# see--/speech_recognition

Measured on AMD Instinct MI355X. Metric: 1s 16kHz clips/sec training throughput, higher is better.
Workload: dtype f32

## Files before the change

include/kws_hip.h:

```cpp
#ifndef KWS_HIP_H_
#define KWS_HIP_H_

#include <stdint.h>

#ifdef __cplusplus
extern "C" {
#endif
#if defined(__GNUC__) || defined(__clang__)
#pragma GCC visibility push(default)
#endif

#define KWS_OK 0
#define KWS_E_INVALID (-1)
#define KWS_E_HIP (-2)
#define KWS_E_WORKSPACE (-3)

#define KWS_ABI_VERSION 5

int kws_abi_version(void);
const char* kws_last_error(void);
int kws_device_name(char* buf, int cap);

int kws_stream_create(int cls, void** stream);
int kws_stream_destroy(void* stream);
// ... 165 lines not shown
                         const float* moving_var, float eps, int C, float* bn, void* stream);
int kws_bn_relu6_apply(const float* y, const float* bn, float* out, int64_t rows, int C, int relu6,
                       void* stream);

int kws_dwconv_fwd_f32(const float* y, const float* bn, const float* w, float* z, int B, int L_in,
                       int L_out, int C, int stride, int pad_l, void* stream);
int64_t kws_dwconv_bwd_part_floats(int B, int L_in, int C);
int kws_dwconv_bwd_f32(const float* dz, const float* y, const float* bn, const float* w, float* g,
                       float* part, int B, int L_in, int L_out, int C, int stride, int pad_l,
                       void* stream);
int kws_dwconv_bwd_bn_f32(const float* dz, const float* y, const float* bn, const float* w,
                          const float* coef, float* dy, float* part, int pass, int B, int L_in,
                          int L_out, int C, int stride, int pad_l, void* stream);
int kws_dw_bwd_finalize(const float* part, int n_parts, int64_t count, int C, float* dw,
                        float* dgamma, float* dbeta, float* coef, float* scratch, void* stream);
int kws_bn_bwd_apply(float* g, const float* y, const float* bn, const float* gamma,
                     const float* coef, int64_t rows, int C, void* stream);

int kws_dwconvk_fwd_f32(const float* y, const float* bn, const float* w, float* z, int B, int L_in, int L_out, int C,
                        int k, int stride, int pad_l, void* stream);
int kws_dwconvk_bwd_part_rows(int B, int L_in, int C, int k, int stride);
int64_t kws_dwconvk_bwd_part_floats(int B, int L_in, int C, int k, int stride);
int kws_dwconvk_bwd_f32(const float* dz, const float* y, const float* bn, const float* w, float* g, float* part, int B,
                        int L_in, int L_out, int C, int k, int stride, int pad_l, void* stream);
int kws_dwconvk_bwd_finalize(const float* part, int n_parts, int64_t count, int C, int k, float* dw, float* dgamma,
                             float* dbeta, float* coef, void* stream);
int kws_dwconvk_pw1_stats_rows(int64_t M);
int kws_dwconvk_pw1_fwd_f32(const float* z, const float* p, float* y, int64_t M, int N, float* stats_part, void* stream);
int64_t kws_dwconvk_pw1_bwd_workspace_floats(int64_t M, int N);
int kws_dwconvk_pw1_bwd_f32(const float* dy, const float* z, const float* p, float* dz, float* dp, int64_t M, int N,
// ... 110 lines not shown
```

speech_recognition_amd/_lib.py:

```python
import ctypes
import os

_HERE = os.path.dirname(os.path.abspath(__file__))
LIB_PATH = os.environ.get("KWS_LIB_PATH") or os.path.join(_HERE, "libkws_hip.so")

ABI_VERSION = 5

KWS_NET_TS_ATTENTION = 1
KWS_NET_LOG_MFCC = 2
KWS_NET_STEFFE = 3
KWS_NET_RESIDUAL = 4
KWS_NET_MFCC_AND_RAW = 5
KWS_NET_CONV_1D_FAST = 6
KWS_NET_CONV_1D_SPEC = 7
KWS_NET_CONV_1D_TIME_STACKED = 8
KWS_NET_CONV_1D_HEAVY = 9
KWS_NET_CONV_1D_GRU = 10
KWS_NET_CONV_1D_MULTI_TIME_SLICED = 11
KWS_NET_CONV_1D_SIMPLE = 12
KWS_NET_XCEPTION_ATTENTION = 13


class KwsError(RuntimeError):
    pass
# ... 141 lines not shown
    "kws_gru_fwd_f32": (_I, [_P] * 12 + [_I, _I, _I, _I, _P]),
    "kws_gru_bwd_f32": (_I, [_P] * 17 + [_I, _I, _I, _I, _P]),
    "kws_attn_gate_fwd_floats": (_I64, [_I, _I, _I, _I]),
    "kws_attn_gate_bwd_floats": (_I64, [_I, _I, _I, _I]),
    "kws_attn_gate_fwd_f32": (_I, [_P] * 12 + [_I, _I, _I, _I, _I, _P]),
    "kws_attn_gate_bwd_f32": (_I, [_P] * 14 + [_I, _I, _I, _I, _I, _P]),
    "kws_transpose_f32": (_I, [_P, _P, _I, _I, _P]),
    "kws_bn_stats_finalize": (_I, [_P, _I, _I64, _I, _P, _P, _F, _F, _P, _P, _P, _P, _P]),
    "kws_bn_infer_prepare": (_I, [_P, _P, _P, _P, _F, _I, _P, _P]),
    "kws_bn_relu6_apply": (_I, [_P, _P, _P, _I64, _I, _I, _P]),
    "kws_dwconv_fwd_f32": (_I, [_P, _P, _P, _P, _I, _I, _I, _I, _I, _I, _P]),
    "kws_dwconv_bwd_part_floats": (_I64, [_I, _I, _I]),
    "kws_dwconv_bwd_f32": (_I, [_P, _P, _P, _P, _P, _P, _I, _I, _I, _I, _I, _I, _P]),
    "kws_dwconv_bwd_bn_f32": (_I, [_P, _P, _P, _P, _P, _P, _P, _I, _I, _I, _I, _I, _I, _I, _P]),
    "kws_dw_bwd_finalize": (_I, [_P, _I, _I64, _I, _P, _P, _P, _P, _P, _P]),
    "kws_bn_bwd_apply": (_I, [_P, _P, _P, _P, _P, _I64, _I, _P]),
    "kws_rmsprop_step": (_I, [_P, _P, _P, _P, _I64, _F, _F, _F, _F, _P]),
    "kws_sgd_momentum_step": (_I, [_P, _P, _P, _P, _I64, _F, _F, _F, _P]),
    "kws_adam_step": (_I, [_P, _P, _P, _P, _P, _I64, _F, _F, _F, _F, _F, _P]),
    "kws_l2_loss": (_I, [_P, _P, _I64, _P, _P]),
    "kws_net_create": (_I, [ctypes.POINTER(NetConfig), ctypes.POINTER(_P)]),
    "kws_net_destroy": (_I, [_P]),
    "kws_net_num_params": (_I64, [_P]),
    "kws_net_num_state": (_I64, [_P]),
    "kws_net_num_tensors": (_I, [_P]),
    "kws_net_tensor_info": (_I, [_P, _I, ctypes.POINTER(TensorInfo)]),
    "kws_net_workspace_bytes": (_I64, [_P, _I, _I]),
    "kws_net_debug_view": (_I, [_P, _I, _I, _I, _I, ctypes.POINTER(_I64), ctypes.POINTER(_I64)]),
    "kws_net_predict": (_I, [_P, _P, _P, _P, _I, _P, _P, _I64, _P]),
    "kws_net_train_fwd_bwd": (_I, [_P, _P, _P, _P, _P, _I, _P, _P, _P, ctypes.c_uint64, ctypes.c_uint32,
# ... 122 lines not shown
```

speech_recognition_amd/csrc/bn.hip:

```cpp
#include "internal.h"

namespace {

constexpr int FIN_CG = 16, FIN_RG = 16;
#ifndef KWS_FIN_U
#define KWS_FIN_U 16
#endif
constexpr int FIN_U = KWS_FIN_U;

__device__ float g_zero_fin[8] = {0.f, 0.f, 0.f, 0.f, 0.f, 0.f, 0.f, 0.f};

__global__ __launch_bounds__(256) void bn_stats_finalize_kernel(const float* __restrict__ part, int n_tiles,
                                                                double inv_count, int C,
                                                                const float* __restrict__ gamma,
                                                                const float* __restrict__ beta, float eps,
                                                                float one_minus_momentum, float* moving_mean,
                                                                float* moving_var, float* __restrict__ bn) {
  __shared__ double red[2][FIN_RG][FIN_CG];
  const int cg = threadIdx.x % FIN_CG, rg = threadIdx.x / FIN_CG;
  const int c = blockIdx.x * FIN_CG + cg;
  double s = 0.0, ss = 0.0;
  if (c < C) {
    for (int t = rg; t < n_tiles; t += FIN_U * FIN_RG) {
      float a[FIN_U], b[FIN_U];
// ... 138 lines not shown
    for (int q = 0; q < 5; ++q) {
      double a = 0.0;
      for (int r = 0; r < FIN_RG; ++r) a += red[q][r][cg];
      s[q] = a;
    }
    if (dbeta) dbeta[c] = (float)s[0];
    if (dgamma) dgamma[c] = (float)s[1];
    if (coef) {
      coef[c] = (float)(s[0] * inv_count);
      coef[C + c] = (float)(s[1] * inv_count);
    }
    if (dw) {
      dw[c] = (float)s[2];
      dw[C + c] = (float)s[3];
      dw[2 * C + c] = (float)s[4];
    }
  }
}

struct DwFinBatch {
  const float* part[KWS_DW_FIN_BATCH];
  float* dw[KWS_DW_FIN_BATCH];
  int n_parts[KWS_DW_FIN_BATCH], C[KWS_DW_FIN_BATCH], blk_end[KWS_DW_FIN_BATCH];
  int n;
};
__global__ __launch_bounds__(256) void dw_grad_finalize_batch_kernel(DwFinBatch b) {
  __shared__ double red[3][FIN_RG][FIN_CG];
  int m = 0;
  while (m + 1 < b.n && (int)blockIdx.x >= b.blk_end[m]) ++m;
  const int blk = blockIdx.x - (m ? b.blk_end[m - 1] : 0);
// ... 154 lines not shown

int kws_dw_bwd_finalize(const float* part, int n_parts, int64_t count, int C, float* dw, float* dgamma, float* dbeta,
                        float* coef, float* scratch, void* stream) {
  KWS_REQUIRE(part && n_parts > 0 && count > 0 && C > 0, "dw_bwd_finalize: bad arguments");
  KwsProfScope prof("bn_finalize", 0.0, 20.0 * n_parts * C, (hipStream_t)stream);
#ifdef KWS_ABL_NO_FIN
  return KWS_OK;
#endif
  KWS_TRY(pre_reduce(part, n_parts, 5 * C, scratch, (hipStream_t)stream, &part, &n_parts));
  hipLaunchKernelGGL(dw_bwd_finalize_kernel, dim3((unsigned)ceil_div(C, FIN_CG)), dim3(FIN_CG * FIN_RG), 0, (hipStream_t)stream, part,
                     n_parts, 1.0 / (double)count, C, dw, dgamma, dbeta, coef);
  KWS_LAUNCH_CHECK("dw_bwd_finalize_kernel");
  return KWS_OK;
}

int kws_bn_bwd_apply(float* g, const float* y, const float* bn, const float* gamma, const float* coef, int64_t rows,
                     int C, void* stream) {
  return kws_bn_bwd_apply_amax(g, y, bn, gamma, coef, rows, C, nullptr, (hipStream_t)stream);
}

int kws_bn_bwd_apply_amax(float* g, const float* y, const float* bn, const float* gamma, const float* coef, int64_t rows,
                          int C, unsigned* amax, void* stream_) {
  hipStream_t stream = (hipStream_t)stream_;
  KWS_REQUIRE(g && y && bn && gamma && coef && rows > 0 && C > 0 && C % 4 == 0, "bn_bwd_apply: bad arguments");
  const int64_t n4 = rows * C / 4;
  KwsProfScope prof("bn_bwd_apply", 6.0 * rows * C, 12.0 * rows * C, (hipStream_t)stream);
  hipLaunchKernelGGL(bn_bwd_apply_kernel, dim3((unsigned)ceil_div64(n4, 256)), dim3(256), 0, (hipStream_t)stream, g, y,
                     bn, gamma, coef, n4, C, amax);
  KWS_LAUNCH_CHECK("bn_bwd_apply_kernel");
  return KWS_OK;
// ... 4 lines not shown
```

speech_recognition_amd/csrc/dw_bwd_body.h:

```cpp
#pragma once
#include "internal.h"

namespace kws_dw {

#ifndef KWS_DW_NT
#define KWS_DW_NT 1
#endif
typedef float dw_v4f __attribute__((ext_vector_type(4)));
__device__ __forceinline__ float4 ld4_stream(const float* p) {
  if (KWS_DW_NT & 2) {
    const dw_v4f v = __builtin_nontemporal_load(reinterpret_cast<const dw_v4f*>(p));
    return make_float4(v.x, v.y, v.z, v.w);
  }
  return *reinterpret_cast<const float4*>(p);
}
__device__ __forceinline__ void st4_stream(float* p, float4 o) {
  if (KWS_DW_NT & 1) {
    dw_v4f v = {o.x, o.y, o.z, o.w};
    __builtin_nontemporal_store(v, reinterpret_cast<dw_v4f*>(p));
    return;
  }
  *reinterpret_cast<float4*>(p) = o;
}

// ... 10 lines not shown
}
__device__ __forceinline__ float4 f4_zero() { return make_float4(0.f, 0.f, 0.f, 0.f); }

#ifndef DW_BWD_THREADS
#define DW_BWD_THREADS 512
#endif
#ifndef DW_BWD_HT
#define DW_BWD_HT 8
#endif
#ifndef DW_BWD2_THREADS
#define DW_BWD2_THREADS 512
#endif
#ifndef DW_BWD_PARTS
#define DW_BWD_PARTS 256
#endif

struct BwdArgs {
  const float* dz; const float* y; const float* bn; const float* w; const float* coef;
  float* g; float* part;
  int B, Lin, Lout, C, pad_l, nchunks, R, Cb;
  unsigned* amax;
  int add_stride = 0, add_len = 0;
};
constexpr int bwd_smem_floats(int mode, int threads) { return mode == 2 ? 4 : 5 * threads * 4; }

template <int S, bool HAS_BN, int MODE, bool GUARD, bool ADDS = false>
__device__ __forceinline__ void bwd_body(const BwdArgs& p, float* const red, const int bid, const int nblk, const int by) {
  const float* __restrict__ dz = p.dz;
  const float* __restrict__ y = p.y;
  const float* __restrict__ bn = p.bn;
  const float* __restrict__ w = p.w;
  const float* __restrict__ coef = p.coef;
  float* __restrict__ g = p.g;
  float* __restrict__ part = p.part;
  const int B = p.B, Lin = p.Lin, Lout = p.Lout, C = p.C, pad_l = p.pad_l, nchunks = p.nchunks, R = p.R, Cb = p.Cb;
  constexpr int RSTRIDE = (MODE == 2 ? 4 : DW_BWD_THREADS * 4);
  float gmax = 0.f;
  const int C4 = Cb >> 2;
  const int tid = threadIdx.x;
  const bool live = !GUARD || tid < R * C4;
  const int r = live ? tid / C4 : 0, c4 = live ? tid - r * C4 : 0;
  const int c = by * Cb + c4 * 4;
  float4 sg = f4_zero(), sgx = f4_zero(), sw0 = f4_zero(), sw1 = f4_zero(), sw2 = f4_zero();
  float4 sc = f4_zero(), sh = f4_zero(), mean = f4_zero(), rstd = f4_zero();
  if (HAS_BN) {
    sc = *reinterpret_cast<const float4*>(bn + c);
    sh = *reinterpret_cast<const float4*>(bn + C + c);
    mean = *reinterpret_cast<const float4*>(bn + 2 * C + c);
    rstd = *reinterpret_cast<const float4*>(bn + 3 * C + c);
  }
  const float4 w0 = *reinterpret_cast<const float4*>(w + c);
  const float4 w1 = *reinterpret_cast<const float4*>(w + C + c);
  const float4 w2 = *reinterpret_cast<const float4*>(w + 2 * C + c);
  float4 c1 = f4_zero(), c2 = f4_zero();
  if (MODE == 2) {
    c1 = *reinterpret_cast<const float4*>(coef + c);
    c2 = *reinterpret_cast<const float4*>(coef + C + c);
  }
  for (int64_t ub = bid; ub * R < (int64_t)B * nchunks; ub += nblk) {
    const int64_t unit = ub * R + r;
    const int64_t b = unit / nchunks;
    const int chunk = (int)(unit - b * nchunks);
    if (b >= B || !live) continue;
    const float* yb = y + b * (int64_t)Lin * C + c;
    float* gb = g + b * (int64_t)Lin * C + c;
    const float* dzb = dz + b * (int64_t)Lout * C + c;
    const int u0 = chunk * TT;
    constexpr int HT = DW_BWD_HT;
    constexpr int ND = S == 1 ? HT + 2 : HT / 2 + 2;
    const bool podd = (pad_l & 1) != 0;
#pragma unroll
    for (int h = 0; h < TT / HT; ++h) {
      const int ub = u0 + h * HT;
      if (ub >= Lin) break;
      float4 yv[HT], D[ND];
#pragma unroll
      for (int i = 0; i < HT; ++i) yv[i] = ld4_stream(yb + (int64_t)(ub + i < Lin ? ub + i : ub) * C);
      const int t_lo = S == 1 ? ub + pad_l - 2 : ((ub + pad_l) >> 1) - 1;
#pragma unroll
      for (int j = 0; j < ND; ++j) {
        const int t = t_lo + j;
        D[j] = ld4_stream(dzb + (int64_t)(t < 0 ? 0 : (t < Lout ? t : Lout - 1)) * C);
      }
// ... 11 lines not shown
          d0 = D[i + 2]; d1 = D[i + 1]; d2 = D[i];
        } else if ((i & 1) == 0) {
          d0 = podd ? f4_zero() : D[i / 2 + 1];
          d2 = podd ? f4_zero() : D[i / 2];
          d1 = podd ? D[i / 2 + 1] : f4_zero();
        } else {
          d0 = podd ? D[(i + 1) / 2 + 1] : f4_zero();
          d2 = podd ? D[(i + 1) / 2] : f4_zero();
          d1 = podd ? f4_zero() : D[(i - 1) / 2 + 1];
        }
        const float4 yy = yv[i];
        float4 a = yy, mk = make_float4(1.f, 1.f, 1.f, 1.f), xh = f4_zero();
        if (HAS_BN) {
          const float4 pre = make_float4(fmaf(yy.x, sc.x, sh.x), fmaf(yy.y, sc.y, sh.y), fmaf(yy.z, sc.z, sh.z),
                                         fmaf(yy.w, sc.w, sh.w));
          a = make_float4(relu6f(pre.x), relu6f(pre.y), relu6f(pre.z), relu6f(pre.w));
          mk = make_float4((pre.x > 0.f && pre.x <= 6.f) ? 1.f : 0.f, (pre.y > 0.f && pre.y <= 6.f) ? 1.f : 0.f,
                           (pre.z > 0.f && pre.z <= 6.f) ? 1.f : 0.f, (pre.w > 0.f && pre.w <= 6.f) ? 1.f : 0.f);
          xh = make_float4((yy.x - mean.x) * rstd.x, (yy.y - mean.y) * rstd.y, (yy.z - mean.z) * rstd.z,
                           (yy.w - mean.w) * rstd.w);
        }
        float4 da = f4_mul(w0, d0);
        da = f4_fma(w1, d1, da);
        da = f4_fma(w2, d2, da);
        const float4 gv = f4_mul(da, mk);
        if (MODE == 2) {
          float4 o;
          o.x = sc.x * (gv.x - c1.x - (yy.x - mean.x) * rstd.x * c2.x);
          o.y = sc.y * (gv.y - c1.y - (yy.y - mean.y) * rstd.y * c2.y);
          o.z = sc.z * (gv.z - c1.z - (yy.z - mean.z) * rstd.z * c2.z);
          o.w = sc.w * (gv.w - c1.w - (yy.w - mean.w) * rstd.w * c2.w);
          st4_stream(gb + (int64_t)u * C, o);
          gmax = kws_abs4max(gmax, o);
          continue;
        }
        if (MODE == 0) {
          float4 o = gv;
          if (coef != nullptr) {
            if (!ADDS) {
              const float4 ad = *reinterpret_cast<const float4*>(coef + (b * (int64_t)Lin + u) * C + c);
              o = make_float4(o.x + ad.x, o.y + ad.y, o.z + ad.z, o.w + ad.w);
            } else {
              const int q = u / p.add_stride;
              const bool on = q * p.add_stride == u && q < p.add_len;
              const float4 ad = *reinterpret_cast<const float4*>(coef + (b * (int64_t)p.add_len + (on ? q : 0)) * C + c);
              o = make_float4(on ? o.x + ad.x : o.x, on ? o.y + ad.y : o.y, on ? o.z + ad.z : o.z, on ? o.w + ad.w : o.w);
            }
          }
          st4_stream(gb + (int64_t)u * C, o);
        }
        sg.x += gv.x; sg.y += gv.y; sg.z += gv.z; sg.w += gv.w;
        sgx = f4_fma(gv, xh, sgx);
        sw0 = f4_fma(d0, a, sw0);
        sw1 = f4_fma(d1, a, sw1);
        sw2 = f4_fma(d2, a, sw2);
      }
    }
  }
  if (MODE == 2) {
    if (p.amax && live) kws_absmax_commit(p.amax, gmax);
    return;
  }
  if constexpr (MODE != 2) {
  if (live) {
    *reinterpret_cast<float4*>(&red[0 * RSTRIDE + tid * 4]) = sg;
    *reinterpret_cast<float4*>(&red[1 * RSTRIDE + tid * 4]) = sgx;
    *reinterpret_cast<float4*>(&red[2 * RSTRIDE + tid * 4]) = sw0;
    *reinterpret_cast<float4*>(&red[3 * RSTRIDE + tid * 4]) = sw1;
    *reinterpret_cast<float4*>(&red[4 * RSTRIDE + tid * 4]) = sw2;
  }
  __syncthreads();
  for (int o = tid; o < 5 * Cb; o += blockDim.x) {
    const int q = o / Cb, ch = o - q * Cb;
    float s = 0.f;
    for (int rr = 0; rr < R; ++rr) s += red[q * RSTRIDE + (rr * C4) * 4 + ch];
    part[((int64_t)bid * 5 + q) * C + by * Cb + ch] = s;
  }
  }
}

constexpr int KWS_DW_BWD_MAX_PARTS = DW_BWD_PARTS;
struct BwdGeom {
  int nchunks, R, block, ny, Cb;
  int64_t grid;
};
inline bool bwd_geom_ok(int C) { return C > 0 && C % 4 == 0 && (C / 4) % ceil_div(C / 4, 256) == 0; }
inline BwdGeom bwd_geom(int B, int Lin, int C, bool parts = true) {
  BwdGeom g;
  const int threads = parts ? DW_BWD_THREADS : DW_BWD2_THREADS;
  const int max_parts = parts ? KWS_DW_BWD_MAX_PARTS : 1024;
  g.ny = ceil_div(C / 4, 256);
  g.Cb = C / g.ny;
  const int C4 = g.Cb / 4;
  g.nchunks = ceil_div(Lin, TT);
  g.R = threads / C4;
  if (g.R < 1) g.R = 1;
  g.block = g.R * C4;
  g.grid = ceil_div64((int64_t)B * g.nchunks, g.R);
  if (g.grid > max_parts) g.grid = max_parts;
  return g;
}

}
```

speech_recognition_amd/csrc/dwconv.hip:

```cpp
#include "dw_bwd_body.h"

namespace {
using namespace kws_dw;

#ifndef DW_FWD_GRID
#define DW_FWD_GRID 4096
#endif

template <int S, bool HAS_BN>
__global__ __launch_bounds__(256) void dwconv_fwd_kernel(const float* __restrict__ y, const float* __restrict__ bn,
                                                         const float* __restrict__ w, float* __restrict__ z,
                                                         int B, int Lin, int Lout, int C, int pad_l, int nchunks,
                                                         unsigned* amax) {
  const int C4 = C >> 2;
  float zmax = 0.f;
  const int64_t total = (int64_t)B * nchunks * C4;
  for (int64_t id = (int64_t)blockIdx.x * 256 + threadIdx.x; id < total; id += (int64_t)gridDim.x * 256) {
    const int c4 = (int)(id % C4);
    const int64_t rest = id / C4;
    const int chunk = (int)(rest % nchunks);
    const int64_t b = rest / nchunks;
    const int c = c4 * 4;
    float4 sc = f4_zero(), sh = f4_zero();
    if (HAS_BN) {
// ... 34 lines not shown
      o = f4_fma(w1, av[S * i + 1], o);
      o = f4_fma(w2, av[S * i + 2], o);
      st4_stream(zb + (int64_t)t * C, o);
      zmax = kws_abs4max(zmax, o);
    }
  }
  if (amax) kws_absmax_commit(amax, zmax);
}

#ifndef KWS_DW_BWD2_MINW
#define KWS_DW_BWD2_MINW 1
#endif
#ifndef KWS_DW_BWD1_MINW
#define KWS_DW_BWD1_MINW 1
#endif
template <int S, bool HAS_BN, int MODE, bool ADDS = false>
__global__ __launch_bounds__(MODE == 2 ? DW_BWD2_THREADS : DW_BWD_THREADS, MODE == 2 ? KWS_DW_BWD2_MINW : KWS_DW_BWD1_MINW) void dwconv_bwd_kernel(BwdArgs p) {
  __shared__ float red[bwd_smem_floats(MODE, DW_BWD_THREADS)];
  bwd_body<S, HAS_BN, MODE, false, ADDS>(p, red, (int)blockIdx.x, (int)gridDim.x, (int)blockIdx.y);
}

}


namespace {
template <int MODE>
int launch_dw_bwd(const float* dz, const float* y, const float* bn, const float* w, const float* coef, float* g,
                  float* part, int B, int L_in, int L_out, int C, int stride, int pad_l, hipStream_t st,
                  unsigned* amax = nullptr, int add_stride = 0, int add_len = 0) {
  const BwdGeom ge = bwd_geom(B, L_in, C, MODE != 2);
  KWS_REQUIRE(ge.grid < 0x7FFFFFFF, "dwconv_bwd: grid too large");
  dim3 gr((unsigned)ge.grid, (unsigned)ge.ny), b((unsigned)ge.block);
  BwdArgs a;
  a.dz = dz; a.y = y; a.bn = bn; a.w = w; a.coef = coef; a.g = g; a.part = part;
  a.B = B; a.Lin = L_in; a.Lout = L_out; a.C = C; a.pad_l = pad_l; a.nchunks = ge.nchunks; a.R = ge.R; a.Cb = ge.Cb; a.amax = amax;
  a.add_stride = add_stride; a.add_len = add_len;
  if (MODE == 0 && add_stride > 1) {
    if (stride == 1) hipLaunchKernelGGL((dwconv_bwd_kernel<1, false, MODE, true>), gr, b, 0, st, a);
    else hipLaunchKernelGGL((dwconv_bwd_kernel<2, false, MODE, true>), gr, b, 0, st, a);
    KWS_LAUNCH_CHECK("dwconv_bwd_kernel");
    return KWS_OK;
  }
  if (stride == 1) {
    if (bn) hipLaunchKernelGGL((dwconv_bwd_kernel<1, true, MODE>), gr, b, 0, st, a);
    else hipLaunchKernelGGL((dwconv_bwd_kernel<1, false, MODE>), gr, b, 0, st, a);
  } else {
    if (bn) hipLaunchKernelGGL((dwconv_bwd_kernel<2, true, MODE>), gr, b, 0, st, a);
    else hipLaunchKernelGGL((dwconv_bwd_kernel<2, false, MODE>), gr, b, 0, st, a);
  }
  KWS_LAUNCH_CHECK("dwconv_bwd_kernel");
  return KWS_OK;
}
}

extern "C" {

int kws_dwconv_fwd_f32(const float* y, const float* bn, const float* w, float* z, int B, int L_in, int L_out,
// ... 75 lines not shown
                               unsigned* amax, void* stream_) {
  hipStream_t stream = (hipStream_t)stream_;
  KWS_REQUIRE(dz && y && bn && w, "dwconv_bwd_bn: NULL pointer");
  KWS_REQUIRE(pass == 1 ? part != nullptr : (pass == 2 && coef != nullptr && dy != nullptr),
              "dwconv_bwd_bn: pass %d needs %s", pass, pass == 1 ? "part" : "coef and dy");
  KWS_REQUIRE(B > 0 && L_in > 0 && L_out > 0 && bwd_geom_ok(C),
              "dwconv_bwd_bn: bad shape B=%d L=%d->%d C=%d", B, L_in, L_out, C);
  KWS_REQUIRE(stride == 1 || stride == 2, "dwconv_bwd_bn: stride %d unsupported", stride);
  hipStream_t st = (hipStream_t)stream;
  KwsProfScope prof("dwconv_bwd", 12.0 * B * L_in * C,
                    4.0 * ((pass == 2 ? 2.0 : 1.0) * B * L_in * C + (double)B * L_out * C), st);
  if (pass == 1) return launch_dw_bwd<1>(dz, y, bn, w, nullptr, nullptr, part, B, L_in, L_out, C, stride, pad_l, st);
  return launch_dw_bwd<2>(dz, y, bn, w, coef, dy, nullptr, B, L_in, L_out, C, stride, pad_l, st, amax);
}

}
```

speech_recognition_amd/csrc/internal.h:

```cpp
#pragma once
#include "common.h"

struct kws_ts_tail_args {
  const float* y; const float* bn; const float* W1; const float* b1; const float* W2; const float* labels;
  float* probs; float* g; float* part; float* xd; float* fd; float* dl1; float* dl2; float* per_loss;
  float* per_correct; float* att; int B, T, C, NC; uint64_t seed; uint32_t step; float keep_prob; float label_smoothing;
  int loss_batch; int64_t row_offset; int train;
};
int kws_ts_tail_launch(const kws_ts_tail_args* p, hipStream_t st);
constexpr int KWS_SMALL_WGRAD_SLICES = 32;
int kws_small_wgrad_launch(const float* X, const float* D, float* out, float* out_bias, int B, int K, int N,
                           float* scratch, hipStream_t st);
int kws_metrics_launch(const float* per_loss, const float* per_correct, int B, float* metrics, hipStream_t st);
struct kws_tail_post_args {
  const float* X2; const float* D2; float* ws2; int K2, N2;
  const float* X1; const float* D1; float* ws1; int K1, N1;
  float* bias1;
  const float* per_loss; const float* per_correct; float* metrics;
  int B;
};
int kws_tail_post_launch(const kws_tail_post_args* a, int* S_out, hipStream_t st);
bool kws_conv1_supported(const kws_gather_t* g, const kws_gather_t* unfolded, int N);
int kws_conv1_stats_rows(int64_t M);
int kws_conv1_fwd(const float* x, const kws_gather_t* g, const kws_gather_t* unfolded, const float* W, float* y, int B, int N,
                  float* stats, hipStream_t st);
int64_t kws_conv1_wgrad_workspace_floats(int64_t M);
int kws_conv1_wgrad(const float* x, const kws_gather_t* g, const kws_gather_t* unfolded, const float* G, float* dW, int B,
                    int N, float* workspace, hipStream_t st);
int kws_conv1_wgrad_slabs(const float* x, const kws_gather_t* g, const kws_gather_t* unfolded, const float* G, float* dW, int B,
                          int N, float* workspace, const float* const* sl_ws, float* const* sl_out, const int64_t* sl_n,
                          const int* sl_S, int n_sl, hipStream_t st);
extern "C" int kws_reduce_slab_groups_f32(float* ws, int64_t n, int S, int per_group, hipStream_t st);
extern "C" int kws_reduce_slabs_f32(const float* ws, float* out, int64_t n, int S, hipStream_t st);
extern "C" int kws_dwconv_bwd_acc_f32(const float* dz, const float* y, const float* w, const float* add, float* g, float* part,
                                      int B, int L_in, int L_out, int C, int stride, int pad_l, hipStream_t st);
extern "C" int kws_dwconv_bwd_acc_strided_f32(const float* dz, const float* y, const float* w, const float* add, int add_stride, int add_len,
                                              float* g, float* part, int B, int L_in, int L_out, int C, int stride, int pad_l, hipStream_t st);
constexpr int KWS_SLAB_BATCH = 16;
extern "C" int kws_gemm_tn_slabs_f32(const float* A, const float* G, int64_t M, int K, int N, float* workspace, int* S,
                                     hipStream_t stream);
extern "C" int kws_gemm_dgrad_wgrad_f32(const float* dY, const float* WT, float* dZ, const float* Z, int64_t M, int cin, int cout,
                                        float* workspace, int* S, hipStream_t stream);
extern "C" bool kws_gather_strided_rows(const kws_gather_t* g, int* lda);
extern "C" int kws_gemm_nn_strided_f32(const float* A, int lda, const float* W, float* C, int64_t M, int K, int N, float* stats_part,
                                       hipStream_t stream);
extern "C" int kws_gemm_tn_slabs_strided_f32(const float* A, int lda, const float* G, int64_t M, int K, int N, float* workspace, int* S,
                                             hipStream_t stream);
extern "C" int kws_gemm_tn_gather_slabs_f32(const float* X, const kws_gather_t* g, const float* G, int B, int N, float* workspace, int* S,
                                            hipStream_t stream);
extern "C" int kws_reduce_slabs_batch(const float* const* ws, float* const* out, const int64_t* n, const int* S, int count,
                                      hipStream_t stream);
extern "C" int64_t kws_gemm_tn_workspace_floats(int64_t M, int K, int N);
struct SlabBatch {
// ... 58 lines not shown
      const float4 v2 = w[(int64_t)(k + 8) * n4 + i], v3 = w[(int64_t)(k + 12) * n4 + i];
      kws_add4(s0, v0); kws_add4(s1, v1); kws_add4(s2, v2); kws_add4(s3, v3);
    }
    for (; k < S; k += 4) kws_add4(s0, w[(int64_t)k * n4 + i]);
    kws_add4(s0, s1); kws_add4(s2, s3); kws_add4(s0, s2);
  }
  red[grp][col] = s0;
  __syncthreads();
  if (grp == 0 && i < n4) {
    float4 r = red[0][col];
    kws_add4(r, red[1][col]); kws_add4(r, red[2][col]); kws_add4(r, red[3][col]);
    reinterpret_cast<float4*>(b.out[m])[i] = r;
  }
}
#endif
struct KwsSlabQueue {
  const float* ws[KWS_SLAB_BATCH];
  float* out[KWS_SLAB_BATCH];
  int64_t n[KWS_SLAB_BATCH];
  int S[KWS_SLAB_BATCH];
  int count = 0;
  float* base = nullptr;
  int64_t used = 0, cap = 0;
  bool allow_pair = true;
  int flush(hipStream_t st) {
    if (count == 0) return 0;
    const int rc = kws_reduce_slabs_batch(ws, out, n, S, count, st);
    count = 0;
    used = 0;
    return rc;
  }
  int gemm(const float* A, const float* G, float* dW, int64_t M, int K, int N, hipStream_t st) {
    const int64_t need = (kws_gemm_tn_workspace_floats(M, K, N) + 63) / 64 * 64;
    if (count == KWS_SLAB_BATCH || used + need > cap) {
      const int rc = flush(st);
      if (rc) return rc;
    }
    if (need > cap) return KWS_E_WORKSPACE;
    ws[count] = base + used; out[count] = dW; n[count] = (int64_t)K * N;
    const int rc = kws_gemm_tn_slabs_f32(A, G, M, K, N, base + used, &S[count], st);
    if (rc) return rc;
    used += need;
    ++count;
    return 0;
  }
  int gemm_gather(const float* X, const kws_gather_t* g, const float* G, float* dW, int B, int N, hipStream_t st) {
    const int64_t M = (int64_t)B * g->L_out;
    const int K = g->taps * g->cin;
    const int64_t need = (kws_gemm_tn_workspace_floats(M, K, N) + 63) / 64 * 64;
    if (count == KWS_SLAB_BATCH || used + need > cap) {
      const int rc = flush(st);
      if (rc) return rc;
    }
    if (need > cap) return KWS_E_WORKSPACE;
    ws[count] = base + used; out[count] = dW; n[count] = (int64_t)K * N;
    int S_ = 0, lda = 0;
    if (kws_gather_strided_rows(g, &lda)) {
      const int rs = kws_gemm_tn_slabs_strided_f32(X, lda, G, M, K, N, base + used, &S_, st);
      if (rs < 0) return rs;
      if (rs == 0) {
        S[count] = S_;
        used += need;
        ++count;
        return 0;
      }
    }
    const int rc = kws_gemm_tn_gather_slabs_f32(X, g, G, B, N, base + used, &S_, st);
    if (rc) return rc;
    S[count] = -S_;
    used += need;
    ++count;
    return 0;
  }
  int pair(const float* dY, const float* WT, float* dZ, const float* Z, float* dW, int64_t M, int cin, int cout, hipStream_t st) {
    const int64_t need = (kws_gemm_tn_workspace_floats(M, cin, cout) + 63) / 64 * 64;
    if (count == KWS_SLAB_BATCH || used + need > cap) {
      const int rc = flush(st);
      if (rc) return rc;
    }
    if (need > cap) return KWS_E_WORKSPACE;
    const int rc = allow_pair ? kws_gemm_dgrad_wgrad_f32(dY, WT, dZ, Z, M, cin, cout, base + used, &S[count], st) : 1;
    if (rc < 0) return rc;
    if (rc == 0) {
      ws[count] = base + used; out[count] = dW; n[count] = (int64_t)cin * cout;
      used += need;
      ++count;
      return 0;
    }
    const int rc2 = kws_gemm_nn_f32(dY, WT, dZ, M, cout, cin, nullptr, st);
    if (rc2) return rc2;
    return gemm(Z, dY, dW, M, cin, cout, st);
// ... 39 lines not shown
```

speech_recognition_amd/csrc/net.hip:

```cpp
#include "net_internal.h"
#include <atomic>
#include <math.h>
#include <stdlib.h>

int64_t kws_net_add_tensor(kws_net* n, const std::string& name, std::vector<int64_t> shape, bool is_state, float l2,
                           int fan_in, int fan_out, float init) {
  kws_tensor_info_t t;
  memset(&t, 0, sizeof(t));
  snprintf(t.name, sizeof(t.name), "%s", name.c_str());
  int64_t size = 1;
  t.ndim = (int)shape.size();
  for (int i = 0; i < t.ndim; ++i) {
    t.shape[i] = shape[i];
    size *= shape[i];
  }
  t.size = size;
  t.is_state = is_state ? 1 : 0;
  t.l2 = l2;
  t.fan_in = fan_in;
  t.fan_out = fan_out;
  t.init = init;
  int64_t& cursor = is_state ? n->n_state : n->n_params;
  t.offset = cursor;
  cursor += (size + 3) / 4 * 4;
// ... 189 lines not shown
  const int n = K1f * C1;
  hipLaunchKernelGGL(fold_taps_kernel, dim3(ceil_div(n, 256)), dim3(256), 0, st, params + conv1, w1f, g.taps, g.cin,
                     g.stride_j, K1f, C1);
  KWS_LAUNCH_CHECK("fold_taps_kernel");
  return KWS_OK;
}
int TsProgram::unfold_conv1(const float* g1f, float* grads, hipStream_t st) const {
  const kws_gather_t& g = gather1;
  const int n = g.taps * g.cin * C1;
  hipLaunchKernelGGL(unfold_taps_kernel, dim3(ceil_div(n, 256)), dim3(256), 0, st, g1f, grads + conv1, g.taps, g.cin,
                     g.stride_j, C1);
  KWS_LAUNCH_CHECK("unfold_taps_kernel");
  return KWS_OK;
}

void TsProgram::make_layout(int B, bool training, Layout* lo) const {
  Bump bp;
  const int nb = (int)blocks.size();
  lo->y.assign(nb + 1, 0);
  lo->z.assign(nb, 0);
  int64_t max_y = (int64_t)B * L1 * C1, max_z = 0, max_part = 0, max_dwpart = 0, max_tn = 0;
  int maxC = C1;
  max_part = std::max((int64_t)kws_gemm_num_row_tiles((int64_t)B * L1), (int64_t)kws_conv1_stats_rows((int64_t)B * L1)) *
             2 * C1;
  max_tn = std::max(kws_gemm_tn_workspace_floats((int64_t)B * L1, K1f, C1),
                    kws_conv1_wgrad_workspace_floats((int64_t)B * L1));
  for (int i = 0; i < nb; ++i) {
    const Block& b = blocks[i];
    const int64_t M = (int64_t)B * b.Lout;
    if (M * b.cout > max_y) max_y = M * b.cout;
// ... 276 lines not shown
  KWS_TRY(kws_small_wgrad_launch(t.xd, t.dl1, grads + d1k, grads + d1b, B, T * C, T,
                                 ws + lo.swg, st));
  }
  {
    const BnRef& r = blocks[nb - 1].bn;
    KWS_TRY(kws_dw_bwd_finalize(part, B, (int64_t)B * T, r.C, nullptr, grads + r.gamma,
                                grads + r.beta, coef, red, st));
  }
  }
  if (run_head) KWS_TRY(transpose_all());
  float* Gb[2] = {ws + lo.G, ws + lo.G2};
  const float* sl_ws[KWS_SLAB_BATCH];
  float* sl_out[KWS_SLAB_BATCH];
  int64_t sl_n[KWS_SLAB_BATCH];
  int sl_S[KWS_SLAB_BATCH], n_sl = 0;
  KWS_REQUIRE(nb + 2 <= KWS_SLAB_BATCH, "net: %d blocks exceed the slab batch", nb);
  if (tail_S > 0) {
    sl_ws[n_sl] = ws + lo.swg; sl_out[n_sl] = grads + d2k; sl_n[n_sl] = (int64_t)2 * C * NC; sl_S[n_sl] = -tail_S; ++n_sl;
    sl_ws[n_sl] = ws + lo.swg1; sl_out[n_sl] = grads + d1k; sl_n[n_sl] = (int64_t)T * C * T; sl_S[n_sl] = -tail_S; ++n_sl;
  }
  const int i_hi = phase == 2 ? split - 1 : nb - 1, i_lo = phase == 1 ? split : 0;
  for (int i = i_hi; i >= i_lo; --i) {
    const Block& b = blocks[i];
    const int64_t M = (int64_t)B * b.Lout;
    float* Gcur = Gb[(i + 1) % 2];
    float* Gnext = Gb[i % 2];
    if (i == nb - 1)
      KWS_TRY(kws_bn_bwd_apply_amax(Gcur, ws + lo.y[i + 1], bn_at(i + 1), params + b.bn.gamma, coef, M, b.cout,
                                    h2 ? g_slots(i) : nullptr, st));
    bool paired = false;
    if (pair_bwd) {
// ... 7 lines not shown
    }
    if (!paired) {
    if (h2 && kws_gemm_nn_f16x2_supported(M, b.cout, b.cin))
      KWS_TRY(kws_gemm_nn_f16x2_f32(Gcur, ws + lo.WPd[i], DZ, M, b.cout, b.cin, g_slots(i), w_slots(i), nullptr, st));
    else
      KWS_TRY(kws_gemm_nn_f32(Gcur, ws + lo.WT[i], DZ, M, b.cout, b.cin, nullptr, st));
    if (h2 && kws_gemm_tn_f16x2_supported(M, b.cin, b.cout))
      KWS_TRY(kws_gemm_tn_f16x2_f32(ws + lo.z[i], Gcur, grads + b.pw, M, b.cin, b.cout, z_slots(i), g_slots(i), ws + lo.tn, st));
    else {
      sl_ws[n_sl] = ws + lo.tns[i]; sl_out[n_sl] = grads + b.pw; sl_n[n_sl] = (int64_t)b.cin * b.cout;
      KWS_TRY(kws_gemm_tn_slabs_f32(ws + lo.z[i], Gcur, M, b.cin, b.cout, ws + lo.tns[i], &sl_S[n_sl], st));
      ++n_sl;
    }
    }
    const BnRef& prev = (i == 0) ? bn1 : blocks[i - 1].bn;
    KWS_TRY(kws_dwconv_bwd_bn_f32(DZ, ws + lo.y[i], bn_at(i), params + b.dw, nullptr, nullptr, part, 1, B, b.Lin, b.Lout,
                                  b.cin, b.stride, b.pad_l, st));
    const int n_parts = (int)(kws_dwconv_bwd_part_floats(B, b.Lin, b.cin) / (5 * b.cin));
    KWS_TRY(kws_dw_bwd_finalize(part, n_parts, (int64_t)B * b.Lin, b.cin, grads + b.dw,
                                grads + prev.gamma, grads + prev.beta, coef, red, st));
    KWS_TRY(kws_dwconv_bwd_bn_amax_f32(DZ, ws + lo.y[i], bn_at(i), params + b.dw, coef, Gnext, nullptr, 2, B, b.Lin, b.Lout,
                                       b.cin, b.stride, b.pad_l, (h2 && i > 0) ? g_slots(i - 1) : nullptr, st));
  }
  const bool sum_with_conv1 = n_sl > 0 && phase != 1 && kws_conv1_supported(&gather1f, &gather1, C1) &&
                              kws_net_get_gemm_mode(net) != 1;
  if (n_sl > 0 && !sum_with_conv1) KWS_TRY(kws_reduce_slabs_batch(sl_ws, sl_out, sl_n, sl_S, n_sl, st));
  if (phase != 1) {
    const int64_t M = (int64_t)B * L1;
    (void)M;
    if (kws_conv1_supported(&gather1f, &gather1, C1)) {
      KWS_TRY(kws_conv1_wgrad_slabs(x, &gather1f, &gather1, Gb[0], grads + conv1, B, C1, ws + lo.tn,
                                    sl_ws, sl_out, sl_n, sl_S, sum_with_conv1 ? n_sl : 0, st));
    } else {
      KWS_TRY(kws_gemm_tn_gather_f32(x, &gather1f, Gb[0], ws + lo.g1f, B, C1, ws + lo.tn, st));
      KWS_TRY(unfold_conv1(ws + lo.g1f, grads, st));
    }
  }
// ... 123 lines not shown
```

Measured before the change: 233,900.

## Split depthwise-conv backward into lean BN-stat pass and fused dgrad+weight-grad pass

For small enough layers, the depthwise conv backward drops from a five-sum stats pass plus a separate dgrad pass to two kernels. A lean pass 3 computes only the two BN reduction sums, without relu6 activation recompute. Pass 4 writes dgrad and also accumulates the three weight-tap sums into per-block rows stored in the freed z buffer. Those rows are reduced later in the existing batched slab reduction, and the slab batch capacity is doubled to hold the extra entries. The aim is to cut redundant reductions and shared-memory traffic in the stats pass and the finalize cost, at the price of more register pressure in the dgrad kernel and a wider slab-reduction batch.

```diff
diff --git a/include/kws_hip.h b/include/kws_hip.h
--- a/include/kws_hip.h
+++ b/include/kws_hip.h
@@ -203,6 +203,13 @@
                           int L_out, int C, int stride, int pad_l, void* stream);
 int kws_dw_bwd_finalize(const float* part, int n_parts, int64_t count, int C, float* dw,
                         float* dgamma, float* dbeta, float* coef, float* scratch, void* stream);
+int kws_dwconv_bwd_rows(int B, int L_in, int C, int pass);
+int kws_dwconv_bwd_bn2_f32(const float* dz, const float* y, const float* bn, const float* w,
+                           const float* coef, float* dy, float* part, int pass, int B, int L_in,
+                           int L_out, int C, int stride, int pad_l, unsigned* amax, void* stream);
+int kws_dw_bwd_finalize2(const float* part, int n_parts, int64_t count, int C, float* dgamma,
+                         float* dbeta, float* coef, float* scratch, void* stream);
+int kws_dw_tap_rows_sum(const float* rows, int n_rows, int C, float* dw, void* stream);
 int kws_bn_bwd_apply(float* g, const float* y, const float* bn, const float* gamma,
                      const float* coef, int64_t rows, int C, void* stream);
 
diff --git a/speech_recognition_amd/_lib.py b/speech_recognition_amd/_lib.py
--- a/speech_recognition_amd/_lib.py
+++ b/speech_recognition_amd/_lib.py
@@ -179,6 +179,10 @@
     "kws_dwconv_bwd_f32": (_I, [_P, _P, _P, _P, _P, _P, _I, _I, _I, _I, _I, _I, _P]),
     "kws_dwconv_bwd_bn_f32": (_I, [_P, _P, _P, _P, _P, _P, _P, _I, _I, _I, _I, _I, _I, _I, _P]),
     "kws_dw_bwd_finalize": (_I, [_P, _I, _I64, _I, _P, _P, _P, _P, _P, _P]),
+    "kws_dwconv_bwd_rows": (_I, [_I, _I, _I, _I]),
+    "kws_dwconv_bwd_bn2_f32": (_I, [_P, _P, _P, _P, _P, _P, _P, _I, _I, _I, _I, _I, _I, _I, _P, _P]),
+    "kws_dw_bwd_finalize2": (_I, [_P, _I, _I64, _I, _P, _P, _P, _P, _P]),
+    "kws_dw_tap_rows_sum": (_I, [_P, _I, _I, _P, _P]),
     "kws_bn_bwd_apply": (_I, [_P, _P, _P, _P, _P, _I64, _I, _P]),
     "kws_rmsprop_step": (_I, [_P, _P, _P, _P, _I64, _F, _F, _F, _F, _P]),
     "kws_sgd_momentum_step": (_I, [_P, _P, _P, _P, _I64, _F, _F, _F, _P]),
diff --git a/speech_recognition_amd/csrc/bn.hip b/speech_recognition_amd/csrc/bn.hip
--- a/speech_recognition_amd/csrc/bn.hip
+++ b/speech_recognition_amd/csrc/bn.hip
@@ -176,6 +176,48 @@
       dw[c] = (float)s[2];
       dw[C + c] = (float)s[3];
       dw[2 * C + c] = (float)s[4];
+    }
+  }
+}
+
+__global__ __launch_bounds__(256) void dw_bwd_finalize2_kernel(const float* __restrict__ part, int n_parts, double inv_count, int C,
+                                                               float* dgamma, float* dbeta, float* coef) {
+  __shared__ double red[2][FIN_RG][FIN_CG];
+  const int cg = threadIdx.x % FIN_CG, rg = threadIdx.x / FIN_CG;
+  const int c = blockIdx.x * FIN_CG + cg;
+  double s[2] = {0, 0};
+  if (c < C) {
+    for (int t = rg; t < n_parts; t += FIN_U * FIN_RG) {
+      float a[FIN_U][2];
+#pragma unroll
+      for (int u = 0; u < FIN_U; ++u) {
+        const int tt = t + u * FIN_RG;
+        const bool ok = tt < n_parts;
+        const float* src = ok ? part + (int64_t)tt * 2 * C + c : g_zero_fin;
+#pragma unroll
+        for (int q = 0; q < 2; ++q) a[u][q] = src[ok ? q * C : q];
+      }
+#pragma unroll
+      for (int u = 0; u < FIN_U; ++u)
+#pragma unroll
+        for (int q = 0; q < 2; ++q) s[q] += (double)a[u][q];
+    }
+  }
+#pragma unroll
+  for (int q = 0; q < 2; ++q) red[q][rg][cg] = s[q];
+  __syncthreads();
+  if (rg == 0 && c < C) {
+#pragma unroll
+    for (int q = 0; q < 2; ++q) {
+      double a = 0.0;
+      for (int r = 0; r < FIN_RG; ++r) a += red[q][r][cg];
+      s[q] = a;
+    }
+    if (dbeta) dbeta[c] = (float)s[0];
+    if (dgamma) dgamma[c] = (float)s[1];
+    if (coef) {
+      coef[c] = (float)(s[0] * inv_count);
+      coef[C + c] = (float)(s[1] * inv_count);
     }
   }
 }
@@ -360,6 +402,20 @@
   return KWS_OK;
 }
 
+int kws_dw_bwd_finalize2(const float* part, int n_parts, int64_t count, int C, float* dgamma, float* dbeta, float* coef,
+                         float* scratch, void* stream) {
+  KWS_REQUIRE(part && n_parts > 0 && count > 0 && C > 0, "dw_bwd_finalize2: bad arguments");
+  KwsProfScope prof("bn_finalize", 0.0, 8.0 * n_parts * C, (hipStream_t)stream);
+#ifdef KWS_ABL_NO_FIN
+  return KWS_OK;
+#endif
+  KWS_TRY(pre_reduce(part, n_parts, 2 * C, scratch, (hipStream_t)stream, &part, &n_parts));
+  hipLaunchKernelGGL(dw_bwd_finalize2_kernel, dim3((unsigned)ceil_div(C, FIN_CG)), dim3(FIN_CG * FIN_RG), 0, (hipStream_t)stream, part,
+                     n_parts, 1.0 / (double)count, C, dgamma, dbeta, coef);
+  KWS_LAUNCH_CHECK("dw_bwd_finalize2_kernel");
+  return KWS_OK;
+}
+
 int kws_bn_bwd_apply(float* g, const float* y, const float* bn, const float* gamma, const float* coef, int64_t rows,
                      int C, void* stream) {
   return kws_bn_bwd_apply_amax(g, y, bn, gamma, coef, rows, C, nullptr, (hipStream_t)stream);
diff --git a/speech_recognition_amd/csrc/dw_bwd_body.h b/speech_recognition_amd/csrc/dw_bwd_body.h
--- a/speech_recognition_amd/csrc/dw_bwd_body.h
+++ b/speech_recognition_amd/csrc/dw_bwd_body.h
@@ -48,6 +48,13 @@
 #ifndef DW_BWD_PARTS
 #define DW_BWD_PARTS 256
 #endif
+#ifndef DW_BWD3_HT
+#define DW_BWD3_HT DW_BWD_HT
+#endif
+#ifndef DW_BWD4_THREADS
+#define DW_BWD4_THREADS 512
+#endif
+constexpr int bwd_threads(int mode) { return mode == 2 ? DW_BWD2_THREADS : mode == 4 ? DW_BWD4_THREADS : DW_BWD_THREADS; }
 
 struct BwdArgs {
   const float* dz; const float* y; const float* bn; const float* w; const float* coef;
@@ -56,7 +63,8 @@
   unsigned* amax;
   int add_stride = 0, add_len = 0;
 };
-constexpr int bwd_smem_floats(int mode, int threads) { return mode == 2 ? 4 : 5 * threads * 4; }
+constexpr int bwd_row_sums(int mode) { return mode == 2 ? 0 : mode == 3 ? 2 : mode == 4 ? 3 : 5; }
+constexpr int bwd_smem_floats(int mode, int threads) { return mode == 2 ? 4 : bwd_row_sums(mode) * threads * 4; }
 
 template <int S, bool HAS_BN, int MODE, bool GUARD, bool ADDS = false>
 __device__ __forceinline__ void bwd_body(const BwdArgs& p, float* const red, const int bid, const int nblk, const int by) {
@@ -68,7 +76,7 @@
   float* __restrict__ g = p.g;
   float* __restrict__ part = p.part;
   const int B = p.B, Lin = p.Lin, Lout = p.Lout, C = p.C, pad_l = p.pad_l, nchunks = p.nchunks, R = p.R, Cb = p.Cb;
-  constexpr int RSTRIDE = (MODE == 2 ? 4 : DW_BWD_THREADS * 4);
+  constexpr int RSTRIDE = (MODE == 2 ? 4 : bwd_threads(MODE) * 4);
   float gmax = 0.f;
   const int C4 = Cb >> 2;
   const int tid = threadIdx.x;
@@ -87,7 +95,7 @@
   const float4 w1 = *reinterpret_cast<const float4*>(w + C + c);
   const float4 w2 = *reinterpret_cast<const float4*>(w + 2 * C + c);
   float4 c1 = f4_zero(), c2 = f4_zero();
-  if (MODE == 2) {
+  if (MODE == 2 || MODE == 4) {
     c1 = *reinterpret_cast<const float4*>(coef + c);
     c2 = *reinterpret_cast<const float4*>(coef + C + c);
   }
@@ -100,7 +108,7 @@
     float* gb = g + b * (int64_t)Lin * C + c;
     const float* dzb = dz + b * (int64_t)Lout * C + c;
     const int u0 = chunk * TT;
-    constexpr int HT = DW_BWD_HT;
+    constexpr int HT = MODE == 3 ? DW_BWD3_HT : DW_BWD_HT;
     constexpr int ND = S == 1 ? HT + 2 : HT / 2 + 2;
     const bool podd = (pad_l & 1) != 0;
 #pragma unroll
@@ -142,7 +150,7 @@
         if (HAS_BN) {
           const float4 pre = make_float4(fmaf(yy.x, sc.x, sh.x), fmaf(yy.y, sc.y, sh.y), fmaf(yy.z, sc.z, sh.z),
                                          fmaf(yy.w, sc.w, sh.w));
-          a = make_float4(relu6f(pre.x), relu6f(pre.y), relu6f(pre.z), relu6f(pre.w));
+          if (MODE != 3) a = make_float4(relu6f(pre.x), relu6f(pre.y), relu6f(pre.z), relu6f(pre.w));
           mk = make_float4((pre.x > 0.f && pre.x <= 6.f) ? 1.f : 0.f, (pre.y > 0.f && pre.y <= 6.f) ? 1.f : 0.f,
                            (pre.z > 0.f && pre.z <= 6.f) ? 1.f : 0.f, (pre.w > 0.f && pre.w <= 6.f) ? 1.f : 0.f);
           xh = make_float4((yy.x - mean.x) * rstd.x, (yy.y - mean.y) * rstd.y, (yy.z - mean.z) * rstd.z,
@@ -152,7 +160,7 @@
         da = f4_fma(w1, d1, da);
         da = f4_fma(w2, d2, da);
         const float4 gv = f4_mul(da, mk);
-        if (MODE == 2) {
+        if (MODE == 2 || MODE == 4) {
           float4 o;
           o.x = sc.x * (gv.x - c1.x - (yy.x - mean.x) * rstd.x * c2.x);
           o.y = sc.y * (gv.y - c1.y - (yy.y - mean.y) * rstd.y * c2.y);
@@ -160,7 +168,7 @@
           o.w = sc.w * (gv.w - c1.w - (yy.w - mean.w) * rstd.w * c2.w);
           st4_stream(gb + (int64_t)u * C, o);
           gmax = kws_abs4max(gmax, o);
-          continue;
+          if (MODE == 2) continue;
         }
         if (MODE == 0) {
           float4 o = gv;
@@ -177,32 +185,42 @@
           }
           st4_stream(gb + (int64_t)u * C, o);
         }
-        sg.x += gv.x; sg.y += gv.y; sg.z += gv.z; sg.w += gv.w;
-        sgx = f4_fma(gv, xh, sgx);
-        sw0 = f4_fma(d0, a, sw0);
-        sw1 = f4_fma(d1, a, sw1);
-        sw2 = f4_fma(d2, a, sw2);
+        if (MODE != 4) {
+          sg.x += gv.x; sg.y += gv.y; sg.z += gv.z; sg.w += gv.w;
+          sgx = f4_fma(gv, xh, sgx);
+        }
+        if (MODE != 3) {
+          sw0 = f4_fma(d0, a, sw0);
+          sw1 = f4_fma(d1, a, sw1);
+          sw2 = f4_fma(d2, a, sw2);
+        }
       }
     }
   }
-  if (MODE == 2) {
+  if (MODE == 2 || MODE == 4) {
     if (p.amax && live) kws_absmax_commit(p.amax, gmax);
-    return;
+    if (MODE == 2) return;
   }
   if constexpr (MODE != 2) {
+  constexpr int NQ = bwd_row_sums(MODE);
   if (live) {
-    *reinterpret_cast<float4*>(&red[0 * RSTRIDE + tid * 4]) = sg;
-    *reinterpret_cast<float4*>(&red[1 * RSTRIDE + tid * 4]) = sgx;
-    *reinterpret_cast<float4*>(&red[2 * RSTRIDE + tid * 4]) = sw0;
-    *reinterpret_cast<float4*>(&red[3 * RSTRIDE + tid * 4]) = sw1;
-    *reinterpret_cast<float4*>(&red[4 * RSTRIDE + tid * 4]) = sw2;
+    int q = 0;
+    if (MODE != 4) {
+      *reinterpret_cast<float4*>(&red[(q++) * RSTRIDE + tid * 4]) = sg;
+      *reinterpret_cast<float4*>(&red[(q++) * RSTRIDE + tid * 4]) = sgx;
+    }
+    if (MODE != 3) {
+      *reinterpret_cast<float4*>(&red[(q++) * RSTRIDE + tid * 4]) = sw0;
+      *reinterpret_cast<float4*>(&red[(q++) * RSTRIDE + tid * 4]) = sw1;
+      *reinterpret_cast<float4*>(&red[(q++) * RSTRIDE + tid * 4]) = sw2;
+    }
   }
   __syncthreads();
-  for (int o = tid; o < 5 * Cb; o += blockDim.x) {
+  for (int o = tid; o < NQ * Cb; o += blockDim.x) {
     const int q = o / Cb, ch = o - q * Cb;
     float s = 0.f;
     for (int rr = 0; rr < R; ++rr) s += red[q * RSTRIDE + (rr * C4) * 4 + ch];
-    part[((int64_t)bid * 5 + q) * C + by * Cb + ch] = s;
+    part[((int64_t)bid * NQ + q) * C + by * Cb + ch] = s;
   }
   }
 }
@@ -213,10 +231,10 @@
   int64_t grid;
 };
 inline bool bwd_geom_ok(int C) { return C > 0 && C % 4 == 0 && (C / 4) % ceil_div(C / 4, 256) == 0; }
-inline BwdGeom bwd_geom(int B, int Lin, int C, bool parts = true) {
+inline BwdGeom bwd_geom(int B, int Lin, int C, int mode = 1) {
   BwdGeom g;
-  const int threads = parts ? DW_BWD_THREADS : DW_BWD2_THREADS;
-  const int max_parts = parts ? KWS_DW_BWD_MAX_PARTS : 1024;
+  const int threads = bwd_threads(mode);
+  const int max_parts = mode != 2 ? KWS_DW_BWD_MAX_PARTS : 1024;
   g.ny = ceil_div(C / 4, 256);
   g.Cb = C / g.ny;
   const int C4 = g.Cb / 4;
diff --git a/speech_recognition_amd/csrc/dwconv.hip b/speech_recognition_amd/csrc/dwconv.hip
--- a/speech_recognition_amd/csrc/dwconv.hip
+++ b/speech_recognition_amd/csrc/dwconv.hip
@@ -72,9 +72,18 @@
 #ifndef KWS_DW_BWD1_MINW
 #define KWS_DW_BWD1_MINW 1
 #endif
+#ifndef KWS_DW_BWD3_MINW
+#define KWS_DW_BWD3_MINW 1
+#endif
+#ifndef KWS_DW_BWD4_MINW
+#define KWS_DW_BWD4_MINW 1
+#endif
+constexpr int bwd_minw(int mode) {
+  return mode == 2 ? KWS_DW_BWD2_MINW : mode == 3 ? KWS_DW_BWD3_MINW : mode == 4 ? KWS_DW_BWD4_MINW : KWS_DW_BWD1_MINW;
+}
 template <int S, bool HAS_BN, int MODE, bool ADDS = false>
-__global__ __launch_bounds__(MODE == 2 ? DW_BWD2_THREADS : DW_BWD_THREADS, MODE == 2 ? KWS_DW_BWD2_MINW : KWS_DW_BWD1_MINW) void dwconv_bwd_kernel(BwdArgs p) {
-  __shared__ float red[bwd_smem_floats(MODE, DW_BWD_THREADS)];
+__global__ __launch_bounds__(bwd_threads(MODE), bwd_minw(MODE)) void dwconv_bwd_kernel(BwdArgs p) {
+  __shared__ float red[bwd_smem_floats(MODE, bwd_threads(MODE))];
   bwd_body<S, HAS_BN, MODE, false, ADDS>(p, red, (int)blockIdx.x, (int)gridDim.x, (int)blockIdx.y);
 }
 
@@ -86,19 +95,25 @@
 int launch_dw_bwd(const float* dz, const float* y, const float* bn, const float* w, const float* coef, float* g,
                   float* part, int B, int L_in, int L_out, int C, int stride, int pad_l, hipStream_t st,
                   unsigned* amax = nullptr, int add_stride = 0, int add_len = 0) {
-  const BwdGeom ge = bwd_geom(B, L_in, C, MODE != 2);
+  const BwdGeom ge = bwd_geom(B, L_in, C, MODE);
   KWS_REQUIRE(ge.grid < 0x7FFFFFFF, "dwconv_bwd: grid too large");
   dim3 gr((unsigned)ge.grid, (unsigned)ge.ny), b((unsigned)ge.block);
   BwdArgs a;
   a.dz = dz; a.y = y; a.bn = bn; a.w = w; a.coef = coef; a.g = g; a.part = part;
   a.B = B; a.Lin = L_in; a.Lout = L_out; a.C = C; a.pad_l = pad_l; a.nchunks = ge.nchunks; a.R = ge.R; a.Cb = ge.Cb; a.amax = amax;
   a.add_stride = add_stride; a.add_len = add_len;
-  if (MODE == 0 && add_stride > 1) {
+  if constexpr (MODE == 0) if (add_stride > 1) {
     if (stride == 1) hipLaunchKernelGGL((dwconv_bwd_kernel<1, false, MODE, true>), gr, b, 0, st, a);
     else hipLaunchKernelGGL((dwconv_bwd_kernel<2, false, MODE, true>), gr, b, 0, st, a);
     KWS_LAUNCH_CHECK("dwconv_bwd_kernel");
     return KWS_OK;
   }
+  if constexpr (MODE == 3 || MODE == 4) {
+    if (stride == 1) hipLaunchKernelGGL((dwconv_bwd_kernel<1, true, MODE>), gr, b, 0, st, a);
+    else hipLaunchKernelGGL((dwconv_bwd_kernel<2, true, MODE>), gr, b, 0, st, a);
+    KWS_LAUNCH_CHECK("dwconv_bwd_kernel");
+    return KWS_OK;
+  } else
   if (stride == 1) {
     if (bn) hipLaunchKernelGGL((dwconv_bwd_kernel<1, true, MODE>), gr, b, 0, st, a);
     else hipLaunchKernelGGL((dwconv_bwd_kernel<1, false, MODE>), gr, b, 0, st, a);
@@ -204,4 +219,29 @@
   return launch_dw_bwd<2>(dz, y, bn, w, coef, dy, nullptr, B, L_in, L_out, C, stride, pad_l, st, amax);
 }
 
-}
+int kws_dwconv_bwd_rows(int B, int L_in, int C, int pass) {
+  if (B <= 0 || L_in <= 0 || !bwd_geom_ok(C) || (pass != 3 && pass != 4)) return 0;
+  return (int)bwd_geom(B, L_in, C, pass).grid;
+}
+
+int kws_dwconv_bwd_bn2_f32(const float* dz, const float* y, const float* bn, const float* w, const float* coef, float* dy,
+                           float* part, int pass, int B, int L_in, int L_out, int C, int stride, int pad_l, unsigned* amax,
+                           void* stream) {
+  KWS_REQUIRE(dz && y && bn && w && part, "dwconv_bwd_bn2: NULL pointer");
+  KWS_REQUIRE(pass == 3 || (pass == 4 && coef != nullptr && dy != nullptr), "dwconv_bwd_bn2: pass %d (3, or 4 with coef and dy)", pass);
+  KWS_REQUIRE(B > 0 && L_in > 0 && L_out > 0 && bwd_geom_ok(C), "dwconv_bwd_bn2: bad shape B=%d L=%d->%d C=%d", B, L_in, L_out, C);
+  KWS_REQUIRE(stride == 1 || stride == 2, "dwconv_bwd_bn2: stride %d unsupported", stride);
+  hipStream_t st = (hipStream_t)stream;
+  KwsProfScope prof("dwconv_bwd", (pass == 3 ? 9.0 : 15.0) * B * L_in * C,
+                    4.0 * ((pass == 4 ? 2.0 : 1.0) * B * L_in * C + (double)B * L_out * C), st);
+  if (pass == 3) return launch_dw_bwd<3>(dz, y, bn, w, nullptr, nullptr, part, B, L_in, L_out, C, stride, pad_l, st);
+  return launch_dw_bwd<4>(dz, y, bn, w, coef, dy, part, B, L_in, L_out, C, stride, pad_l, st, amax);
+}
+
+int kws_dw_tap_rows_sum(const float* rows, int n_rows, int C, float* dw, void* stream) {
+  KWS_REQUIRE(rows && dw && n_rows > 0 && C > 0 && C % 4 == 0, "dw_tap_rows_sum: bad arguments");
+  const int64_t n = 3 * (int64_t)C;
+  return kws_reduce_slabs_batch(&rows, &dw, &n, &n_rows, 1, (hipStream_t)stream);
+}
+
+}
diff --git a/speech_recognition_amd/csrc/internal.h b/speech_recognition_amd/csrc/internal.h
--- a/speech_recognition_amd/csrc/internal.h
+++ b/speech_recognition_amd/csrc/internal.h
@@ -36,7 +36,7 @@
                                       int B, int L_in, int L_out, int C, int stride, int pad_l, hipStream_t st);
 extern "C" int kws_dwconv_bwd_acc_strided_f32(const float* dz, const float* y, const float* w, const float* add, int add_stride, int add_len,
                                               float* g, float* part, int B, int L_in, int L_out, int C, int stride, int pad_l, hipStream_t st);
-constexpr int KWS_SLAB_BATCH = 16;
+constexpr int KWS_SLAB_BATCH = 32;
 extern "C" int kws_gemm_tn_slabs_f32(const float* A, const float* G, int64_t M, int K, int N, float* workspace, int* S,
                                      hipStream_t stream);
 extern "C" int kws_gemm_dgrad_wgrad_f32(const float* dY, const float* WT, float* dZ, const float* Z, int64_t M, int cin, int cout,
@@ -125,6 +125,7 @@
   }
 }
 #endif
+constexpr int KWS_SLAB_QUEUE = 16;
 struct KwsSlabQueue {
   const float* ws[KWS_SLAB_BATCH];
   float* out[KWS_SLAB_BATCH];
@@ -143,7 +144,7 @@
   }
   int gemm(const float* A, const float* G, float* dW, int64_t M, int K, int N, hipStream_t st) {
     const int64_t need = (kws_gemm_tn_workspace_floats(M, K, N) + 63) / 64 * 64;
-    if (count == KWS_SLAB_BATCH || used + need > cap) {
+    if (count == KWS_SLAB_QUEUE || used + need > cap) {
       const int rc = flush(st);
       if (rc) return rc;
     }
@@ -159,7 +160,7 @@
     const int64_t M = (int64_t)B * g->L_out;
     const int K = g->taps * g->cin;
     const int64_t need = (kws_gemm_tn_workspace_floats(M, K, N) + 63) / 64 * 64;
-    if (count == KWS_SLAB_BATCH || used + need > cap) {
+    if (count == KWS_SLAB_QUEUE || used + need > cap) {
       const int rc = flush(st);
       if (rc) return rc;
     }
@@ -185,7 +186,7 @@
   }
   int pair(const float* dY, const float* WT, float* dZ, const float* Z, float* dW, int64_t M, int cin, int cout, hipStream_t st) {
     const int64_t need = (kws_gemm_tn_workspace_floats(M, cin, cout) + 63) / 64 * 64;
-    if (count == KWS_SLAB_BATCH || used + need > cap) {
+    if (count == KWS_SLAB_QUEUE || used + need > cap) {
       const int rc = flush(st);
       if (rc) return rc;
     }
diff --git a/speech_recognition_amd/csrc/net.hip b/speech_recognition_amd/csrc/net.hip
--- a/speech_recognition_amd/csrc/net.hip
+++ b/speech_recognition_amd/csrc/net.hip
@@ -227,6 +227,11 @@
   return KWS_OK;
 }
 
+#ifndef KWS_DW_LEAN_MAX_ELEMS
+#define KWS_DW_LEAN_MAX_ELEMS 14000000ll
+#endif
+static bool dw_bwd_lean(int B, int Lin, int Lout, int C) { return (int64_t)B * (Lin + Lout) * C <= KWS_DW_LEAN_MAX_ELEMS; }
+
 void TsProgram::make_layout(int B, bool training, Layout* lo) const {
   Bump bp;
   const int nb = (int)blocks.size();
@@ -533,7 +538,7 @@
   float* sl_out[KWS_SLAB_BATCH];
   int64_t sl_n[KWS_SLAB_BATCH];
   int sl_S[KWS_SLAB_BATCH], n_sl = 0;
-  KWS_REQUIRE(nb + 2 <= KWS_SLAB_BATCH, "net: %d blocks exceed the slab batch", nb);
+  KWS_REQUIRE(2 * nb + 2 <= KWS_SLAB_BATCH, "net: %d blocks exceed the slab batch", nb);
   if (tail_S > 0) {
     sl_ws[n_sl] = ws + lo.swg; sl_out[n_sl] = grads + d2k; sl_n[n_sl] = (int64_t)2 * C * NC; sl_S[n_sl] = -tail_S; ++n_sl;
     sl_ws[n_sl] = ws + lo.swg1; sl_out[n_sl] = grads + d1k; sl_n[n_sl] = (int64_t)T * C * T; sl_S[n_sl] = -tail_S; ++n_sl;
@@ -571,13 +576,24 @@
     }
     }
     const BnRef& prev = (i == 0) ? bn1 : blocks[i - 1].bn;
-    KWS_TRY(kws_dwconv_bwd_bn_f32(DZ, ws + lo.y[i], bn_at(i), params + b.dw, nullptr, nullptr, part, 1, B, b.Lin, b.Lout,
-                                  b.cin, b.stride, b.pad_l, st));
-    const int n_parts = (int)(kws_dwconv_bwd_part_floats(B, b.Lin, b.cin) / (5 * b.cin));
-    KWS_TRY(kws_dw_bwd_finalize(part, n_parts, (int64_t)B * b.Lin, b.cin, grads + b.dw,
-                                grads + prev.gamma, grads + prev.beta, coef, red, st));
-    KWS_TRY(kws_dwconv_bwd_bn_amax_f32(DZ, ws + lo.y[i], bn_at(i), params + b.dw, coef, Gnext, nullptr, 2, B, b.Lin, b.Lout,
-                                       b.cin, b.stride, b.pad_l, (h2 && i > 0) ? g_slots(i - 1) : nullptr, st));
+    const int n_parts = kws_dwconv_bwd_rows(B, b.Lin, b.cin, 3), n_taps = kws_dwconv_bwd_rows(B, b.Lin, b.cin, 4);
+    if (dw_bwd_lean(B, b.Lin, b.Lout, b.cin) && (int64_t)n_taps * 3 <= M) {
+      float* taps = ws + lo.z[i];
+      KWS_TRY(kws_dwconv_bwd_bn2_f32(DZ, ws + lo.y[i], bn_at(i), params + b.dw, nullptr, nullptr, part, 3, B, b.Lin, b.Lout,
+                                     b.cin, b.stride, b.pad_l, nullptr, st));
+      KWS_TRY(kws_dw_bwd_finalize2(part, n_parts, (int64_t)B * b.Lin, b.cin, grads + prev.gamma, grads + prev.beta, coef, red, st));
+      KWS_TRY(kws_dwconv_bwd_bn2_f32(DZ, ws + lo.y[i], bn_at(i), params + b.dw, coef, Gnext, taps, 4, B, b.Lin, b.Lout,
+                                     b.cin, b.stride, b.pad_l, (h2 && i > 0) ? g_slots(i - 1) : nullptr, st));
+      sl_ws[n_sl] = taps; sl_out[n_sl] = grads + b.dw; sl_n[n_sl] = (int64_t)3 * b.cin; sl_S[n_sl] = n_taps;
+      ++n_sl;
+    } else {
+      KWS_TRY(kws_dwconv_bwd_bn_f32(DZ, ws + lo.y[i], bn_at(i), params + b.dw, nullptr, nullptr, part, 1, B, b.Lin, b.Lout,
+                                    b.cin, b.stride, b.pad_l, st));
+      KWS_TRY(kws_dw_bwd_finalize(part, n_parts, (int64_t)B * b.Lin, b.cin, grads + b.dw,
+                                  grads + prev.gamma, grads + prev.beta, coef, red, st));
+      KWS_TRY(kws_dwconv_bwd_bn_amax_f32(DZ, ws + lo.y[i], bn_at(i), params + b.dw, coef, Gnext, nullptr, 2, B, b.Lin, b.Lout,
+                                         b.cin, b.stride, b.pad_l, (h2 && i > 0) ? g_slots(i - 1) : nullptr, st));
+    }
   }
   const bool sum_with_conv1 = n_sl > 0 && phase != 1 && kws_conv1_supported(&gather1f, &gather1, C1) &&
                               kws_net_get_gemm_mode(net) != 1;
```

New measurement: 233,800. No clear change (-0.0%).
